# mattm458/tacotron2

Measured on AMD Instinct MI355X. Metric: mel-frames/sec (node), LJSpeech-shaped teacher-forced train step, b=32/GPU, fp32, higher is better.
Workload: dtype f32

## Files before the change

### include/tacotron2_amd.h

```cpp
#ifndef TACOTRON2_AMD_H
#define TACOTRON2_AMD_H
#include <stdint.h>
#ifdef __cplusplus
extern "C" {
#endif

#define T2_OK 0
#define T2_ERR_ARG 1
#define T2_ERR_LAUNCH 2
#define T2_ERR_RESIDENCY 3

const char* t2_last_error(void);
int t2_version(void);
int t2_sizeof(const char* struct_name);
int t2_debug_clock(int enable, uint64_t* out8);

typedef struct {
    const float* A; const float* B; float* C;
    int M, N, K;
    int64_t lda, ldb, ldc;
    int a_kmajor, b_kmajor;
    float alpha;
    const float* bias; const float* bias2;
    const float* mulmask; int64_t ldmask;
// ... 105 lines not shown
    const float* pre; const float* pmT; const float* memory; const int32_t* len;
    const float* att_drop;
    float* xdec; float* att_c; float* gates; float* align; float* cum; float* th;
    float* xproj_ctx; int64_t ld_xproj;
    float* e_part;
    int t_begin, t_end;
    float* xdec_t;
    uint64_t* clk;
} T2AttnSeq;
int t2_attn_seq_fwd(const T2AttnSeq* a, void* stream);

typedef struct {
    int B, L, T, A, Ad, Ef, Kl;
    const float* W_ih_ctx; int64_t ld_wih;
    const float* W_hh; const float* Wq; const float* U; const float* v;
    const float* wtp_ctx;
    const float* wtp_h;
    const float* wtp_q;
    const float* memory; const float* xdec; const float* att_c; const float* gates; const float* align;
    const float* cum; const float* th; const float* att_drop;
    const float* dh_ext; int64_t ld_dh;
    const float* dctx_ext1; int64_t ld_dc1;
    const float* dctx_ext2; int64_t ld_dc2;
    float* dgates; float* dctx_tot; float* dq; float* dpmT; float* dv_part; float* dU_part;
    float* dc; float* G; float* de; float* din_part;
    float* dh_rec;
    int t_hi, t_lo;
    float* dgates_t;
    uint64_t* clk;
    float* ws_bd;
    const float* dalign;
} T2AttnSeqBwd;
int t2_attn_seq_bwd(const T2AttnSeqBwd* a, void* stream);

int t2_embedding_fwd(const int64_t* idx, const float* table, float* out, int B, int L, int E, int pad, void* stream);
int t2_embedding_bwd(const int64_t* idx, const float* dout, float* dtable, int B, int L, int E, int Lp, int pad, void* stream);
int t2_pack_conv_weight(const float* w, float* wp, int Co, int Ci, int K, int flip, void* stream);
int t2_unpack_conv_wgrad(const float* gp, float* g, int Co, int Ci, int K, void* stream);

typedef struct {
    int B, L, C;
    const float* x; int Lp_x;
    const float* gamma; const float* beta;
    float* running_mean; float* running_var;
    int training; float momentum, eps;
    double* sums;
    float* mean; float* invstd;
    int act;
    const float* drop;
    const float* res; int Lp_res, pad_res;
    const int32_t* len; float fill;
    float* y; int Lp_y, pad_y;
    const float* dy; int Lp_dy, pad_dy;
    float* dx; int Lp_dx, pad_dx;
    float* dgamma; float* dbeta;
    int phase; const float* shift; float grad_share;
    int sums_prezeroed;
    const float* tile_stats; int tile_M;
} T2Bn;
int t2_bn_fwd(const T2Bn* s, void* stream);
int t2_bn_bwd(const T2Bn* s, void* stream);

int t2_colsum(const float* x, int64_t ld, int64_t R, int C, float* out, void* stream);
int t2_mel_to_tm(const float* mel, float* out, int B, int T, int M, void* stream);
int t2_swap01(const float* in, float* out, int D0, int D1, int C, int accumulate, void* stream);
int t2_finalize_fwd(const float* proj, int64_t ld_proj, const int32_t* len, float* mels, float* gates, float* post_in, int B,
// ... 65 lines not shown
```

### tacotron2_amd/csrc/t2_attention.hip

```cpp
#include "t2_common.hpp"
#include "t2_lstm_step.hpp"

int t2_lstm_step_fwd_launch(const T2LstmStep* steps, int n, hipStream_t st);
int t2_lstm_step_bwd_launch(const T2LstmBwdStep* steps, int n, hipStream_t st, unsigned long long* clk = nullptr);
void t2_lstm_fwd_advance(T2LstmStep& c, const T2LstmStride& inc);
void t2_lstm_bwd_advance(T2LstmBwdStep& c, const T2LstmBwdStride& inc);

namespace {

constexpr int KL = 31, KPAD = 15;

struct AttnK {
    int B, L, A, Ad, Ef;
    const float* att_h; long ldh;
    const float* Wq; const float* U; const float* v;
    const float* w_prev; long ldw; const float* cum_prev; long ldcum;
    const float* pmT; const float* memory; const int32_t* len;
    float* e_part; float* th_out;
    float* w_out; long ldwo; float* cum_out; long ldco;
    float* ctx_out; long ldctx; float* ctx_out2; long ldctx2;
    float* ctxt_out; int ctxt_col0; long ctxt_cs;
    unsigned long long* clk;
    int win_back, win_fwd; int32_t* win_peak;
};
// ... 618 lines not shown
        memset(&q, 0, sizeof(q));
        q.B = B; q.L = L; q.A = A; q.Ad = Ad; q.Ef = Ef; q.Kl = a->Kl;
        q.att_h = slot1; q.ldh = ldx; q.Wq = a->Wq; q.U = a->U; q.v = a->v;
        if (t > 0) { q.w_prev = a->align + (long)(t - 1) * L; q.ldw = (long)T * L; }
        q.cum_prev = a->cum + (long)t * B * L; q.ldcum = L;
        q.pmT = a->pmT; q.memory = a->memory; q.len = a->len; q.e_part = a->e_part;
        if (a->th) q.th_out = a->th + (long)t * B * Ad * ((L + 3) & ~3);
        q.w_out = a->align + (long)t * L; q.ldwo = (long)T * L;
        q.cum_out = a->cum + (long)(t + 1) * B * L; q.ldco = L;
        q.ctx_out = slot1 + A; q.ldctx = ldx;
        if (a->xproj_ctx) { q.ctx_out2 = a->xproj_ctx + (long)t * B * a->ld_xproj; q.ldctx2 = a->ld_xproj; }
        if (a->xdec_t) { q.ctxt_out = a->xdec_t + (long)(t + 1) * xts; q.ctxt_col0 = A; }
        q.clk = a->clk;
        if (t == tb) T2_TRY(check_attn(q));
        T2_TRY(launch_attn(q, st));
    }
    return T2_OK;
}

struct AttnBwdK {
    int B, L, Ad, Ef;
    const float* dctx; long lddctx;
    const float* ctx; long ldctx;
    const float* w; long ldw;
    const float* memory;
    const float* din_part; const float* G_in; float* G_out;
    const float* dalign;
    float* de;
    const float* th; const float* v; const float* U;
    const float* w_prev; long ldwp; const float* cum_prev; long ldcp;
    float* dpmT; float* dq; long lddq; float* dv_part; float* dU_part; float* din_part_out;
    unsigned long long* clk;
    const unsigned* bd;
};

namespace {

__global__ __launch_bounds__(256, 1) void attn_bwd_dw_kernel(AttnBwdK p) {
    T2_CHAIN_PRIO();
    extern __shared__ __attribute__((aligned(16))) float sm[];
    const int b = blockIdx.x, l0 = blockIdx.y * 32, tid = threadIdx.x;
    const int L = p.L, Ef = p.Ef, NA = p.Ad >> 4;
    constexpr int NEV = 20;
    const int DS = imax(Ef, 32 * NEV);
    float* dctx_s = sm;
    float* dwx_s = dctx_s + DS;
    float* red = dwx_s + ((L + 3) & ~3);
    [[maybe_unused]] const bool stamp = b == 0 && blockIdx.y == 0 && tid == 0;
    T2_STAMP(p, stamp, 16);
    T2_RING_BEGIN(p.clk, stamp, 3);
    const int l = l0 + (tid >> 3), sub = tid & 7;
    float dv0[4], cv0[4];
#pragma unroll
    for (int i = 0; i < 4; ++i) {
        const int e = imin(tid + 256 * i, Ef - 1);
        dv0[i] = p.dctx[(long)b * p.lddctx + e];
        cv0[i] = p.ctx[(long)b * p.ldctx + e];
    }
    const int lc0 = imin(tid, L - 1);
    float a0[8], a1[8];
#pragma unroll
    for (int jj = 0; jj < 8; ++jj) { a0[jj] = 0.f; a1[jj] = 0.f; }
    if (p.din_part) {
#pragma unroll
        for (int jj = 0; jj < 8; ++jj) {
            const long o = (((long)b * NA + imin(jj, NA - 1)) * 2) * L + lc0;
// ... 96 lines not shown
}

constexpr int DSH = 25;
constexpr int DS_ONE = 252;
constexpr int DS_TI = 216;
constexpr int DS_MARGIN = 16;

__global__ void attn_bwd_prep_kernel(const float* U, unsigned* bd, int Ad) {
    const int j = blockIdx.x, ks = blockIdx.y, lane = threadIdx.x, n = lane & 15, q = lane >> 4;
    const int blk = 4 * ks + q, al = blk / 5, rb = blk - 5 * al, c = n >> 3, sft = n & 7;
    float v[8];
#pragma unroll
    for (int jj = 0; jj < 8; ++jj) {
        const int k = 32 - (8 * rb + jj) + sft;
        v[jj] = (k >= 0 && k < KL) ? U[((long)(j * 16 + al) * 2 + c) * KL + k] : 0.f;
    }
    const Split8 sp = t2_split8(v);
    u32x4v* o = reinterpret_cast<u32x4v*>(bd) + ((long)(j * 20 + ks) * 3) * 64 + lane;
    o[0] = __builtin_bit_cast(u32x4v, sp.h); o[64] = __builtin_bit_cast(u32x4v, sp.m); o[128] = __builtin_bit_cast(u32x4v, sp.l);
}

struct DsDims { int NG, L4, M8, MT, KS, S16, LpI; };
__host__ __device__ inline DsDims ds_dims(int L) {
    DsDims d;
    d.NG = (L + 3) >> 2; d.L4 = 4 * d.NG; d.M8 = (L + 7) >> 3; d.MT = (d.M8 + 15) >> 4; d.KS = (L + 31) >> 5;
    int g = d.M8 + 5;
    if (4 * d.KS + 4 > g) g = 4 * d.KS + 4;
    if ((DSH + d.L4 + 7) / 8 + 1 > g) g = (DSH + d.L4 + 7) / 8 + 1;
    d.S16 = g | 1;
    d.LpI = 32 * d.KS + 96;
    return d;
}

template <bool TILED>
__device__ __forceinline__ void attn_bwd_ds_mfma_body(const AttnBwdK& p, float* sm) {
    const int b = blockIdx.x, j = blockIdx.y;
    const int tid = threadIdx.x, lane = tid & 63;
    [[maybe_unused]] const bool stamp = b == 0 && j == 0 && tid == 0;
    T2_STAMP(p, stamp, 24);
    T2_RING_BEGIN(p.clk, stamp, 4);
    const int w = __builtin_amdgcn_readfirstlane(tid >> 6);
    const int al = tid >> 5, sub = tid & 31, a = j * 16 + al;
    const int n = lane & 15, q = lane >> 4;
    const int Lg = p.L, Lg4 = (Lg + 3) & ~3;
    const DsDims dm = ds_dims(TILED ? imin(Lg, DS_TI + 2 * DS_MARGIN) : Lg);
    const int S16 = dm.S16, LpI = dm.LpI;
    u32x4v* DX = reinterpret_cast<u32x4v*>(sm);
    unsigned* PX = reinterpret_cast<unsigned*>(DX + 48 * S16);
    float* des = reinterpret_cast<float*>(PX + 6 * LpI);
    float* redC = des + dm.L4 + 8;
    float* dinacc = redC + 4 * 256;
    float* red = reinterpret_cast<float*>(DX);
    const long rowoff = ((long)b * p.Ad + a) * Lg;
    const float va = p.v[a];
    const float* th_base = p.th + ((long)b * p.Ad + a) * Lg4;
    const int c_nt = w & 3, c_c = c_nt >> 1, c_k = 16 * (c_nt & 1) + n;
    float sq = 0.f, sv = 0.f;
    f32x4 ch0 = {0.f, 0.f, 0.f, 0.f}, cl0 = ch0, cl1 = ch0, cl2 = ch0;
    u32x4v bdv[3][3];
    float dv_old = 0.f, dU_old[4] = {0.f, 0.f, 0.f, 0.f};
    const int ntile = TILED ? (Lg + DS_TI - 1) / DS_TI : 1;
    if (TILED) {
        for (int i = tid; i < 2 * Lg4; i += ENT) dinacc[i] = 0.f;
    }
    for (int tile = 0; tile < ntile; ++tile) {
        const int a0 = TILED ? tile * DS_TI : 0, b0 = TILED ? imin(a0 + DS_TI, Lg) : Lg;
        const int v0 = TILED ? imax(a0 - DS_MARGIN, 0) : 0, v1 = TILED ? imin(b0 + DS_MARGIN, Lg) : Lg;
        const int L = v1 - v0, ia = a0 - v0, ib = b0 - v0;
        const DsDims dd = TILED ? ds_dims(L) : dm;
        const int L4 = dd.L4, M8 = dd.M8, MT = dd.MT, KS = dd.KS;
        const int NGA = (L + 4) >> 2;
        float dev[TILED ? 1 : 2];
#pragma unroll
        for (int i = 0; i < (TILED ? 1 : 2); ++i) dev[i] = p.de[(long)b * Lg + v0 + imin(tid + ENT * i, L - 1)];
        float thv[EMAXI][4], dpv[EMAXI][4];
        const float* th_row = th_base + v0;
#pragma unroll
        for (int it = 0; it < EMAXI; ++it) {
            const int g = imin(sub + 32 * it, NGA - 1);
            const f32x4 t4 = *reinterpret_cast<const f32x4*>(th_row + imin(4 * g, L4 - 4));
            thv[it][0] = th_row[imax(4 * g - 1, 0)];
            thv[it][1] = t4[0]; thv[it][2] = t4[1]; thv[it][3] = t4[2];
        }
#pragma unroll
        for (int it = 0; it < EMAXI; ++it) {
            const int g = imin(sub + 32 * it, NGA - 1);
#pragma unroll
            for (int i = 0; i < 4; ++i) dpv[it][i] = p.dpmT[rowoff + v0 + imin(imax(4 * g - 1 + i, 0), L - 1)];
        }
        if (tile == 0) dv_old = p.dv_part[(long)b * p.Ad + a];
        StageRegs<ENT> sr;
        stage_issue<ENT, true, false>(sr, p.w_prev, p.ldwp, p.cum_prev, p.ldcp, p.U, p.dpmT, b, j, Lg, LpI, tid, 40, v0);
        if (tile == 0) {
            const u32x4v* bdp = reinterpret_cast<const u32x4v*>(p.bd) + (long)j * 20 * 3 * 64 + lane;
#pragma unroll
            for (int ki = 0; ki < 3; ++ki) {
                const int ks = imin(w + 8 * ki, 19);
#pragma unroll
                for (int pl = 0; pl < 3; ++pl) bdv[ki][pl] = bdp[(ks * 3 + pl) * 64];
            }
        }
        for (int i = tid; i < 48 * S16; i += ENT) DX[i] = (u32x4v){0u, 0u, 0u, 0u};
        stage_commit_split<ENT, false>(sr, PX, nullptr, p.w_prev, p.ldwp, p.cum_prev, p.ldcp, p.dpmT, b, Lg, LpI, tid, 40, v0);
#pragma unroll
        for (int i = 0; i < (TILED ? 1 : 2); ++i) {
            const int l = tid + ENT * i;
            if (l < dm.L4 + 7) des[l + 1] = (l >= ia && l < ib) ? dev[i] : 0.f;
        }
        if (tid == 0) des[0] = 0.f;
        __syncthreads();
        T2_STAMP(p, stamp, 25);

        {
            uint2* dx64 = reinterpret_cast<uint2*>(DX);
#pragma unroll
            for (int it = 0; it < EMAXI; ++it) {
                const int g = sub + 32 * it;
                if (g >= NGA) continue;
                f32x4 d4 = {0.f, 0.f, 0.f, 0.f};
                const f32x4 de4 = *reinterpret_cast<const f32x4*>(des + 4 * g);
#pragma unroll
                for (int i = 0; i < 4; ++i) {
                    const int l = 4 * g - 1 + i;
                    if (l >= ia && l < ib) {
                        const float th = thv[it][i];
                        d4[i] = de4[i] * va * (1.f - th * th);
                        sv += de4[i] * th;
                        p.dpmT[rowoff + v0 + l] = dpv[it][i] + d4[i];
                    }
                }
                sq += (d4[0] + d4[1]) + (d4[2] + d4[3]);
                const Split3 s3 = split3_attn(d4);
                const int o = al * S16 * 2 + 6 + g;
                dx64[o] = s3.h; dx64[16 * S16 * 2 + o] = s3.m; dx64[32 * S16 * 2 + o] = s3.l;
            }
        }
        if (!TILED) {
            sq = t2_half_sum_hi(sq); sv = t2_half_sum_hi(sv);
            if (sub == 31) {
                p.dq[(long)b * p.lddq + a] = sq;
                p.dv_part[(long)b * p.Ad + a] = dv_old + sv;
            }
        }
        __syncthreads();
        T2_STAMP(p, stamp, 26);
        if (tile == 0 && w < 4 && c_k < KL) {
#pragma unroll
            for (int r = 0; r < 4; ++r) dU_old[r] = p.dU_part[(((long)b * p.Ad + j * 16 + 4 * q + r) * 2 + c_c) * KL + c_k];
        }

        for (int ks = w >> 2; ks < KS + 1; ks += 2) {
            const int it = n * S16 + 4 * ks + q;
            Split8 fa, fb;
            fa.h = __builtin_bit_cast(bf16x8, DX[it]); fa.m = __builtin_bit_cast(bf16x8, DX[16 * S16 + it]); fa.l = __builtin_bit_cast(bf16x8, DX[32 * S16 + it]);
            const unsigned* bp = PX + c_c * LpI + 32 * ks + 8 * q + c_k;
            fb.h = __builtin_bit_cast(bf16x8, (u32x4v){bp[0], bp[2], bp[4], bp[6]});
            fb.m = __builtin_bit_cast(bf16x8, (u32x4v){bp[2 * LpI], bp[2 * LpI + 2], bp[2 * LpI + 4], bp[2 * LpI + 6]});
            fb.l = __builtin_bit_cast(bf16x8, (u32x4v){bp[4 * LpI], bp[4 * LpI + 2], bp[4 * LpI + 4], bp[4 * LpI + 6]});
            cl0 = __builtin_amdgcn_mfma_f32_16x16x32_bf16(fa.l, fb.h, cl0, 0, 0, 0);
            cl1 = __builtin_amdgcn_mfma_f32_16x16x32_bf16(fa.h, fb.l, cl1, 0, 0, 0);
            cl2 = __builtin_amdgcn_mfma_f32_16x16x32_bf16(fa.m, fb.m, cl2, 0, 0, 0);
            cl0 = __builtin_amdgcn_mfma_f32_16x16x32_bf16(fa.m, fb.h, cl0, 0, 0, 0);
            cl1 = __builtin_amdgcn_mfma_f32_16x16x32_bf16(fa.h, fb.m, cl1, 0, 0, 0);
            ch0 = __builtin_amdgcn_mfma_f32_16x16x32_bf16(fa.h, fb.h, ch0, 0, 0, 0);
        }
        if (!TILED && w >= 4) {
            const f32x4 cC1 = ch0 + ((cl0 + cl1) + cl2);
#pragma unroll
            for (int r = 0; r < 4; ++r) redC[c_nt * 256 + (4 * q + r) * 16 + n] = cC1[r];
        }
        T2_STAMP(p, stamp, 28);
        f32x4 cD[2];
#pragma unroll
        for (int mt = 0; mt < 2; ++mt) {
            f32x4 h0 = {0.f, 0.f, 0.f, 0.f}, l0 = h0, l1 = h0, l2 = h0;
            if (mt < MT) {
                const int m = imin(16 * mt + n, M8 - 1);
#pragma unroll
                for (int ki = 0; ki < 3; ++ki) {
                    const int ks = w + 8 * ki;
                    if (ks < 20) {
                        const int blk = 4 * ks + q, ad = blk / 5, rb = blk - 5 * ad;
                        const int it = ad * S16 + m + rb + 1;
                        Split8 fa, fb;
                        fa.h = __builtin_bit_cast(bf16x8, DX[it]); fa.m = __builtin_bit_cast(bf16x8, DX[16 * S16 + it]); fa.l = __builtin_bit_cast(bf16x8, DX[32 * S16 + it]);
                        fb.h = __builtin_bit_cast(bf16x8, bdv[ki][0]); fb.m = __builtin_bit_cast(bf16x8, bdv[ki][1]); fb.l = __builtin_bit_cast(bf16x8, bdv[ki][2]);
                        l0 = __builtin_amdgcn_mfma_f32_16x16x32_bf16(fa.l, fb.h, l0, 0, 0, 0);
                        l1 = __builtin_amdgcn_mfma_f32_16x16x32_bf16(fa.h, fb.l, l1, 0, 0, 0);
                        l2 = __builtin_amdgcn_mfma_f32_16x16x32_bf16(fa.m, fb.m, l2, 0, 0, 0);
                        l0 = __builtin_amdgcn_mfma_f32_16x16x32_bf16(fa.m, fb.h, l0, 0, 0, 0);
                        l1 = __builtin_amdgcn_mfma_f32_16x16x32_bf16(fa.h, fb.m, l1, 0, 0, 0);
                        h0 = __builtin_amdgcn_mfma_f32_16x16x32_bf16(fa.h, fb.h, h0, 0, 0, 0);
                    }
                }
            }
            cD[mt] = h0 + ((l0 + l1) + l2);
        }
        __syncthreads();
        T2_STAMP(p, stamp, 27);
#pragma unroll
        for (int mt = 0; mt < 2; ++mt) {
            if (mt < MT) {
#pragma unroll
                for (int r = 0; r < 4; ++r) red[((w * MT + mt) * 16 + 4 * q + r) * 16 + n] = cD[mt][r];
            }
        }
        if (!TILED && w < 4 && c_k < KL) {
            const f32x4 cC0 = ch0 + ((cl0 + cl1) + cl2);
#pragma unroll
            for (int r = 0; r < 4; ++r)
                p.dU_part[(((long)b * p.Ad + j * 16 + 4 * q + r) * 2 + c_c) * KL + c_k] = dU_old[r] + cC0[r] + redC[c_nt * 256 + (4 * q + r) * 16 + n];
        }
        __syncthreads();
        T2_STAMP(p, stamp, 29);
        for (int o = tid; o < MT * 256; o += ENT) {
            const int mt = o >> 8, ml = (o >> 4) & 15, nn = o & 15;
            float s2 = 0.f;
#pragma unroll
            for (int ww = 0; ww < 8; ++ww) s2 += red[((ww * MT + mt) * 16 + ml) * 16 + nn];
            const int m = 16 * mt + ml, l = 8 * m + (nn & 7);
            if (m < M8 && l < L) {
                if (TILED) dinacc[(nn >> 3) * Lg4 + v0 + l] += s2;
                else p.din_part_out[(((long)b * (p.Ad >> 4) + j) * 2 + (nn >> 3)) * Lg + l] = s2;
            }
        }
        if (TILED) __syncthreads();
    }
    if (TILED) {
        sq = t2_half_sum_hi(sq); sv = t2_half_sum_hi(sv);
        if (sub == 31) {
            p.dq[(long)b * p.lddq + a] = sq;
            p.dv_part[(long)b * p.Ad + a] = dv_old + sv;
        }
    }
    if (TILED) {
        const f32x4 cC = ch0 + ((cl0 + cl1) + cl2);
        if (w >= 4) {
#pragma unroll
            for (int r = 0; r < 4; ++r) redC[c_nt * 256 + (4 * q + r) * 16 + n] = cC[r];
        }
        __syncthreads();
        if (w < 4 && c_k < KL) {
#pragma unroll
            for (int r = 0; r < 4; ++r)
                p.dU_part[(((long)b * p.Ad + j * 16 + 4 * q + r) * 2 + c_c) * KL + c_k] = dU_old[r] + cC[r] + redC[c_nt * 256 + (4 * q + r) * 16 + n];
        }
    }
    if (TILED) {
        for (int i = tid; i < 2 * Lg; i += ENT) {
            const int c = i >= Lg ? 1 : 0, l = i - c * Lg;
            p.din_part_out[(((long)b * (p.Ad >> 4) + j) * 2 + c) * Lg + l] = dinacc[c * Lg4 + l];
        }
    }
    T2_STAMP(p, stamp, 30);
    T2_RING_END();
}

__global__ __launch_bounds__(ENT, 4) void attn_bwd_ds_mfma_kernel(AttnBwdK p) {
    T2_CHAIN_PRIO();
    extern __shared__ __attribute__((aligned(16))) float sm[];
    attn_bwd_ds_mfma_body<false>(p, sm);
}
__global__ __launch_bounds__(ENT, 2) void attn_bwd_ds_tiled_kernel(AttnBwdK p) {
    T2_CHAIN_PRIO();
    extern __shared__ __attribute__((aligned(16))) float sm[];
    attn_bwd_ds_mfma_body<true>(p, sm);
}

size_t ds_mfma_lds(int L) {
    const bool tiled = L > DS_ONE;
    const DsDims dd = ds_dims(tiled ? (L < DS_TI + 2 * DS_MARGIN ? L : DS_TI + 2 * DS_MARGIN) : L);
    size_t f = (size_t)48 * dd.S16 * 4 + 6 * dd.LpI + dd.L4 + 8 + 4 * 256;
    if (tiled) f += (size_t)2 * ((L + 3) & ~3);
    return f * sizeof(float);
}

}

extern "C" int t2_attn_seq_bwd(const T2AttnSeqBwd* a, void* stream) {
    (void)hipGetLastError();
    T2_REQUIRE(a != nullptr, "t2_attn_seq_bwd: null");
    T2_REQUIRE(a->Kl == KL && a->Ad % 16 == 0 && a->Ef % 32 == 0, "t2_attn_seq_bwd: unsupported dims");
    T2_REQUIRE(a->L >= 1, "t2_attn_seq_bwd: need L >= 1");
    T2_REQUIRE(a->ws_bd && a->th, "t2_attn_seq_bwd: the filter workspace ws_bd and the forward's tanh stash th are required");
    hipStream_t st = (hipStream_t)stream;
    const int B = a->B, L = a->L, T = a->T, A = a->A, Ef = a->Ef, Ad = a->Ad, NA = Ad / 16;
    const long ldx = A + Ef;
    const size_t sm_dw = (size_t)((Ef > 640 ? Ef : 640) + ((L + 3) & ~3) + 8) * sizeof(float);
    const bool tiled = L > DS_ONE;
    const size_t sm_dsm = ds_mfma_lds(L);
    T2_REQUIRE(t2_allow_lds(attn_bwd_dw_kernel, sm_dw) && (tiled ? t2_allow_lds(attn_bwd_ds_tiled_kernel, sm_dsm) : t2_allow_lds(attn_bwd_ds_mfma_kernel, sm_dsm)),
               "t2_attn_seq_bwd: the text is too long for the LDS images of the attention backward kernels");
    hipLaunchKernelGGL(attn_bwd_prep_kernel, dim3(NA, 20), dim3(64), 0, st, a->U, reinterpret_cast<unsigned*>(a->ws_bd), Ad);
    T2_REQUIRE(a->wtp_ctx && a->wtp_h, "t2_attn_seq_bwd: packed weight streams (t2_lstm_pack_bwd) are required");
    const long ldz = 4 * A + Ad;
    float* Z = a->dgates;
    T2_REQUIRE(a->wtp_q && a->dh_rec, "t2_attn_seq_bwd: wtp_q / dh_rec required");
    T2_REQUIRE(!a->dgates_t || A % 16 == 0, "t2_attn_seq_bwd: dgates_t needs A % 16 == 0");
    const int thi = (a->t_hi == 0 && a->t_lo == 0) ? T : a->t_hi, tlo = (a->t_hi == 0 && a->t_lo == 0) ? 0 : a->t_lo;
    T2_REQUIRE(tlo >= 0 && thi <= T && tlo <= thi, "t2_attn_seq_bwd: bad frame range");
    T2LstmBwdStep s2[2];
    for (int t = thi - 1; t >= tlo; --t) {
        const bool last = (t == T - 1);
        const float* zrow = Z + (long)(t + 1) * B * ldz;
        memset(s2, 0, sizeof(s2));
        T2LstmBwdStep& s = s2[0];
        s.B = B; s.H = A; s.N4 = 4 * A; s.dg_next = zrow; s.lddg = ldz; s.W = a->W_ih_ctx; s.ldw = a->ld_wih;
        s.ncols = Ef; s.epi = 0; s.wtpacked = a->wtp_ctx;
        s.ext1 = a->dctx_ext1 + (long)t * B * a->ld_dc1; s.ldx1 = a->ld_dc1;
        s.ext2 = a->dctx_ext2 + (long)t * B * a->ld_dc2; s.ldx2 = a->ld_dc2;
        s.dx_out = a->dctx_tot + (long)t * B * Ef; s.lddx = Ef;
        const long zts = (long)(4 * A / 16) * ((B + 15) / 16 * 16) * 16;
        if (a->dgates_t) s.dgt_next = a->dgates_t + (long)(t + 1) * zts;
        T2LstmBwdStep& r = s2[1];
        r.B = B; r.H = A; r.N4 = 4 * A; r.dg_next = zrow; r.lddg = ldz; r.W = a->W_hh; r.ldw = A;
        r.ncols = A; r.epi = 0; r.wtpacked = a->wtp_h;
        r.ext1 = a->dh_ext + (long)t * B * a->ld_dh; r.ldx1 = a->ld_dh;
        r.dx_out = a->dh_rec; r.lddx = A;
        if (a->dgates_t) r.dgt_next = a->dgates_t + (long)(t + 1) * zts;
        T2_TRY(t2_lstm_step_bwd_launch(s2, 2, st, (unsigned long long*)a->clk));
        AttnBwdK k;
        memset(&k, 0, sizeof(k));
        k.B = B; k.L = L; k.Ad = Ad; k.Ef = Ef;
        k.dctx = a->dctx_tot + (long)t * B * Ef; k.lddctx = Ef;
        k.ctx = a->xdec + (long)(t + 1) * B * ldx + A; k.ldctx = ldx;
        k.w = a->align + (long)t * L; k.ldw = (long)T * L;
        k.memory = a->memory;
        k.din_part = last ? nullptr : a->din_part;
        k.G_in = last ? nullptr : a->G + (long)((t + 1) & 1) * B * L;
        k.G_out = a->G + (long)(t & 1) * B * L;
        k.dalign = a->dalign ? a->dalign + (long)t * L : nullptr;
        k.de = a->de;
        k.th = a->th + (long)t * B * Ad * ((L + 3) & ~3); k.v = a->v; k.U = a->U;
        if (t > 0) { k.w_prev = a->align + (long)(t - 1) * L; k.ldwp = (long)T * L; }
        k.cum_prev = a->cum + (long)t * B * L; k.ldcp = L;
        k.dpmT = a->dpmT; k.dq = Z + (long)(t + 1) * B * ldz + 4 * A; k.lddq = ldz;
        k.dv_part = a->dv_part; k.dU_part = a->dU_part; k.din_part_out = a->din_part;
        k.clk = (unsigned long long*)a->clk;
        hipLaunchKernelGGL(attn_bwd_dw_kernel, dim3(B, t2_cdiv(L, 32)), dim3(256), sm_dw, st, k);
        k.bd = reinterpret_cast<const unsigned*>(a->ws_bd);
        if (tiled) hipLaunchKernelGGL(attn_bwd_ds_tiled_kernel, dim3(B, NA), dim3(ENT), sm_dsm, st, k);
        else hipLaunchKernelGGL(attn_bwd_ds_mfma_kernel, dim3(B, NA), dim3(ENT), sm_dsm, st, k);
        T2LstmBwdStep c;
        memset(&c, 0, sizeof(c));
        c.B = B; c.H = A; c.N4 = Ad; c.dg_next = Z + (long)(t + 1) * B * ldz + 4 * A; c.lddg = ldz; c.W = a->Wq; c.ldw = A;
        c.ncols = A; c.epi = 1; c.wtpacked = a->wtp_q;
        c.ext1 = a->dh_rec; c.ldx1 = A;
        if (a->att_drop) { c.drop = a->att_drop + (long)t * B * A; c.lddrop = A; }
        c.gates = a->gates + (long)t * B * 4 * A; c.ldgs = 4 * A;
        c.c_prev = a->att_c + (long)t * B * A; c.ldcp = A;
        c.c_cur = a->att_c + (long)(t + 1) * B * A; c.ldcc = A;
        c.dc = a->dc; c.lddc = A;
        c.dg_out = Z + (long)t * B * ldz; c.ldgo = ldz;
        if (a->dgates_t) c.dgt_out = a->dgates_t + (long)t * zts;
        T2_TRY(t2_lstm_step_bwd_launch(&c, 1, st, (unsigned long long*)a->clk));
    }
    T2_CHECK_LAUNCH();
    return T2_OK;
}
```

### tacotron2_amd/engine.py

```python
from __future__ import annotations

import contextlib
import numbers
import threading as _threading
from typing import Dict, Optional

import torch

from . import _lib
from . import guard as _guard
from ._lib import call, make
from .params import ParamStore

KL, KPAD = 31, 15


def _stream():
    return torch.cuda.current_stream().cuda_stream


_TLS = _threading.local()


@contextlib.contextmanager
# ... 845 lines not shown
        def proj_wgrads():
            self._wgrad(dproj, M + 1, _ptr(xproj, B * ldp), ldp, ps.cat_view("decoder.mel_out.weight", M + 1, ldp, grad=True),
                        ldp, M + 1, ldp, R)
            call("t2_colsum", dproj, M + 1, R, M + 1, ps.cat_view("decoder.mel_out.bias", M + 1, 0, grad=True), _stream())
            if ctl is not None:
                C = ctl.shape[1]
                s_proj = self.buf("ctl.dproj_sum", B, M + 1, zero=True)
                call("t2_colsum", dproj, B * (M + 1), T, B * (M + 1), s_proj, _stream())
                self._wgrad(s_proj, M + 1, ctl, C, G["decoder.mel_out.weight#controls"], C, M, C, B)
        post_wgrads.append(proj_wgrads)

        dgd = self.buf("dgd", T + 1, B, 4 * D)
        zero_later(dgd[T])
        Bp = (B + 15) // 16 * 16
        dgd_t = self.buf("dgd_t", T + 1, 4 * D // 16, Bp, 16)
        zero_later(dgd_t[T])
        Zt = self.buf("Zatt_t", T + 1, 4 * A // 16, Bp, 16)
        zero_later(Zt[T])
        dc_dec = self.buf("dc_dec", B, D, zero=True)
        dd = masks.get("dec_drop")
        wtp_dec = self.pack_bwd("dec.t", P["decoder.lstm.weight_hh"], D, 4 * D, D)
        dxdec = self.buf("dxdec", T, B, ldx)
        ldz = 4 * A + Ad
        Z = self.buf("Zatt", T + 1, B, ldz)
        zero_later(Z[T, :, :4 * A])
        dga = Z
        dctx_tot = self.buf("dctx_tot", T, B, Ef)
        dpmT = self.buf("dpmT", B, Ad, L, zero=True)
        dv_part = self.buf("dv_part", B, Ad, zero=True)
        dU_part = self.buf("dU_part", B, Ad * 2 * KL, zero=True)
        dc_att = self.buf("dc_att", B, A, zero=True)
        Gc = self.buf("Gcum", 2, B, L)
        de = self.buf("de", B, L)
        din_part = self.buf("din_part", B, Ad // 16, 2, L)
        wtp_ctx = self.pack_bwd("att.ctx.t", _ptr(P["decoder.att_rnn.weight_ih"], Pd), Pd + Ef, 4 * A, Ef)
        wtp_h = self.pack_bwd("att.h.t", P["decoder.att_rnn.weight_hh"], A, 4 * A, A)
        wtp_q = self.pack_bwd("att.q.t", P["decoder.attention.query_layer.weight"], A, Ad, A)
        dh_rec = self.buf("dh_rec", B, A)
        sb = make("T2AttnSeqBwd", B=B, L=L, T=T, A=A, Ad=Ad, Ef=Ef, Kl=KL, wtp_ctx=wtp_ctx, wtp_h=wtp_h, wtp_q=wtp_q,
                  dh_rec=dh_rec,
                  W_ih_ctx=_ptr(P["decoder.att_rnn.weight_ih"], Pd), ld_wih=Pd + Ef, W_hh=P["decoder.att_rnn.weight_hh"],
                  Wq=P["decoder.attention.query_layer.weight"], U=ctx["U"], v=P["decoder.attention.v.weight"],
                  memory=ctx["memory"], xdec=xdec, att_c=ctx["att_c"], gates=ctx["gates_att"], align=ctx["align"],
                  cum=ctx["cum"], th=ctx["th"], att_drop=masks.get("att_drop"),
                  dh_ext=dxdec, ld_dh=ldx, dctx_ext1=_ptr(dxdec, A), ld_dc1=ldx, dctx_ext2=_ptr(dxproj, D), ld_dc2=ldp,
                  dgates=Z, dctx_tot=dctx_tot, dq=None, dpmT=dpmT, dv_part=dv_part, dU_part=dU_part,
                  dc=dc_att, G=Gc, de=de, din_part=din_part, dgates_t=Zt, clk=getattr(self, "clk_bwd", None), dalign=d_align,
                  ws_bd=self.buf("attn.ws_bd", Ad // 16 * 16896))
        self.mark("bwd.dec.proj")
        main, side = torch.cuda.current_stream(), self.side_stream()
        self._wait(side, main)
        CH = self.chunk_bwd

        def dec_bwd_chunk(hi, lo):
            s = make("T2LstmBwdStep", B=B, H=D, N4=4 * D, dg_next=_ptr(dgd, hi * B * 4 * D), lddg=4 * D,
                     W=P["decoder.lstm.weight_hh"], ldw=D, wtpacked=wtp_dec, ncols=D, epi=1,
                     ext1=_ptr(dxproj, (hi - 1) * B * ldp), ldx1=ldp,
                     drop=_ptr(dd, (hi - 1) * B * D) if dd is not None else None, lddrop=D,
                     gates=_ptr(ctx["gates_dec"], (hi - 1) * B * 4 * D), ldgs=4 * D,
                     c_prev=_ptr(ctx["dec_c"], (hi - 1) * B * D), ldcp=D, c_cur=_ptr(ctx["dec_c"], hi * B * D), ldcc=D,
                     dc=dc_dec, lddc=D, dg_out=_ptr(dgd, (hi - 1) * B * 4 * D), ldgo=4 * D,
                     dgt_next=_ptr(dgd_t, hi * Bp * 4 * D), dgt_out=_ptr(dgd_t, (hi - 1) * Bp * 4 * D),
                     off_chain=1 if self.bptt_off_chain else 0)
            inc = make("T2LstmBwdStride", dg=-B * 4 * D, ext1=-B * ldp, drop=-B * D, gates=-B * 4 * D, c_prev=-B * D,
                       c_cur=-B * D, dt=0, dgt=-Bp * 4 * D)
            return s, inc

        def dec_wgrads_chunk(hi, lo):
            n = (hi - lo) * B
            g0 = _ptr(dgd, lo * B * 4 * D)
            self._wgrad(g0, 4 * D, _ptr(xdec, (lo + 1) * B * ldx), ldx, G["decoder.lstm.weight_ih"], ldx, 4 * D, ldx, n)
            self._wgrad(g0, 4 * D, _ptr(xproj, lo * B * ldp), ldp, G["decoder.lstm.weight_hh"], D, 4 * D, D, n)

        chunks, hi = [], T
        for n in reversed(_chunk_sizes(T, CH, ramp_at_end=self.ramp_chunks)):
            chunks.append((hi, hi - n)); hi -= n
        gWih = G["decoder.att_rnn.weight_ih"]

        def att_wgrads(hi, lo):
            n = (hi - lo) * B
            z0 = _ptr(Z, lo * B * ldz)
            self._wgrad(z0, ldz, _ptr(ctx["p2"], lo * B * Pd), Pd, gWih, Pd + Ef, 4 * A, Pd, n)
            self._wgrad(z0, ldz, _ptr(xdec, lo * B * ldx + A), ldx, _ptr(gWih, Pd), Pd + Ef, 4 * A, Ef, n)
            self._wgrad(z0, ldz, _ptr(xdec, lo * B * ldx), ldx, G["decoder.att_rnn.weight_hh"], A, 4 * A, A, n)
            self._wgrad(_ptr(Z, (lo + 1) * B * ldz + 4 * A), ldz, _ptr(xdec, (lo + 1) * B * ldx), ldx,
                        G["decoder.attention.query_layer.weight"], A, Ad, A, n)
        WG = max(1, int(self.wgrad_group))
        dec_grp, att_done, att_grp = None, [], None
        for ci_, (hi, lo) in enumerate(chunks):
            with torch.cuda.stream(side), share_cu(self.share_cu):
                s, inc = dec_bwd_chunk(hi, lo)
                call("t2_lstm_seq_bwd", s, inc, 1, hi - lo, side.cuda_stream)
                gemm(_ptr(dgd, lo * B * 4 * D), P["decoder.lstm.weight_ih"], _ptr(dxdec, lo * B * ldx), (hi - lo) * B, ldx, 4 * D,
                     4 * D, ldx, ldx, a_k=1, b_k=0)
                ev = self._record(side)
                dec_grp = [hi, lo, 1] if dec_grp is None else [dec_grp[0], lo, dec_grp[2] + 1]
                if dec_grp[2] >= WG:
                    dec_wgrads_chunk(dec_grp[0], dec_grp[1]); dec_grp = None
                if post_wgrads and ci_ >= 4:
                    post_wgrads.pop(0)()
                if len(att_done) >= 2:
                    h2, l2, e2 = att_done.pop(0)
                    att_grp = [h2, l2, 1, e2] if att_grp is None else [att_grp[0], l2, att_grp[2] + 1, e2]
                    if att_grp[2] >= WG:
                        self._wait(side, att_grp[3])
                        att_wgrads(att_grp[0], att_grp[1]); att_grp = None
            self._wait(main, ev)
            sb.t_hi, sb.t_lo = hi, lo
            call("t2_attn_seq_bwd", sb, st)
            att_done.append((hi, lo, self._record(main)))
        with torch.cuda.stream(side):
            while post_wgrads:
                post_wgrads.pop(0)()
            with share_cu(self.share_cu):
                if dec_grp is not None:
                    dec_wgrads_chunk(dec_grp[0], dec_grp[1])
                for h2, l2, e2 in att_done:
                    att_grp = [h2, l2, 1, e2] if att_grp is None else [att_grp[0], l2, att_grp[2] + 1, e2]
                if att_grp is not None:
                    self._wait(side, att_grp[3])
                    att_wgrads(att_grp[0], att_grp[1])
            db = self.buf("db_dec", 4 * D, zero=True)
            call("t2_colsum", dgd, 4 * D, R, 4 * D, db, side.cuda_stream)
            for nm in ("decoder.lstm.bias_ih", "decoder.lstm.bias_hh"):
                call("t2_colsum", db, 4 * D, 1, 4 * D, G[nm], side.cuda_stream)
            if ctl is not None:
                s_dgd = self.buf("ctl.dgd_sum", B, 4 * D, zero=True)
                call("t2_colsum", dgd, B * 4 * D, T, B * 4 * D, s_dgd, side.cuda_stream)
                self._wgrad(s_dgd, 4 * D, ctl, ctl.shape[1], G["decoder.lstm.weight_ih#controls"], ctl.shape[1], 4 * D,
                            ctl.shape[1], B)
        self.mark("bwd.dec.chains")

        dmem = self.buf("dmem", B, L, Ef)
        gemm(ctx["align"], dctx_tot, dmem, L, Ef, T, L, B * Ef, Ef, a_k=0, b_k=0, batch=B, sA=T * L, sB=Ef, sC=L * Ef)
        Watt = P["att_encoder.weight"]
        gemm(dpmT, Watt, dmem, L, Ef, Ad, L, Ef, Ef, a_k=0, b_k=0, accumulate=1, batch=B, sA=Ad * L, sB=0, sC=L * Ef)

        self._wait(side, main)
        with torch.cuda.stream(side):
            sst = side.cuda_stream
            db = self.buf("db_att", 4 * A, zero=True)
            call("t2_colsum", dga, ldz, R, 4 * A, db, sst)
            for nm in ("decoder.att_rnn.bias_ih", "decoder.att_rnn.bias_hh"):
                call("t2_colsum", db, 4 * A, 1, 4 * A, G[nm], sst)
            call("t2_colsum", dv_part, Ad, B, Ad, G["decoder.attention.v.weight"], sst)
            dU = self.buf("dU", Ad, 2 * KL, zero=True)
            call("t2_colsum", dU_part, Ad * 2 * KL, B, Ad * 2 * KL, dU, sst)
            Wd, Wc = P["decoder.attention.location_dense.weight"], P["decoder.attention.location_conv.weight"]
            gemm(dU, Wc, G["decoder.attention.location_dense.weight"], Ad, F, 2 * KL, 2 * KL, 2 * KL, F, accumulate=1)
            gemm(Wd, dU, G["decoder.attention.location_conv.weight"], F, 2 * KL, Ad, F, 2 * KL, 2 * KL, a_k=0, b_k=0,
                 accumulate=1)
            gemm(dpmT, ctx["memory"], G["att_encoder.weight"], Ad, Ef, L, L, Ef, Ef, a_k=1, b_k=0, accumulate=2, batch=B,
                 sA=Ad * L, sB=L * Ef, sC=0)
            dp2 = self.buf("dp2", T + 1, B, Pd)
            zero_later(dp2[T])
            gemm(dga, P["decoder.att_rnn.weight_ih"], dp2, R, Pd, 4 * A, ldz, Pd + Ef, Pd, a_k=1, b_k=0)
            pd = ctx["pd"]
            g2 = self.buf("g2", T + 1, B, Pd)
            call("t2_relu_mask_bwd", dp2, ctx["p2"], pd[1] if pd else None, g2, R1 * Pd, sst)
            self._wgrad(g2, Pd, ctx["p1"], Pd, G["prenet.3.weight"], Pd, Pd, Pd, R1)
            dp1 = self.buf("dp1", T + 1, B, Pd)
            gemm(g2, P["prenet.3.weight"], dp1, R1, Pd, Pd, Pd, Pd, Pd, a_k=1, b_k=0)
            g1 = self.buf("g1", T + 1, B, Pd)
            call("t2_relu_mask_bwd", dp1, ctx["p1"], pd[0] if pd else None, g1, R1 * Pd, sst)
            self._wgrad(g1, Pd, ctx["mel_tm"], M, G["prenet.0.weight"], M, Pd, M, R1)
            if self.grad_tail_hook is not None:
                self.grad_tail_hook()
        self.mark("bwd.dec.attn_gemms")
# ... 250 lines not shown
```

Measured before the change: 291,900.

## Split attention backward into chain-critical part and deferred side-stream accumulation

The per-frame attention backward kernel on the serial chain is split. A lighter chain variant computes only the recurrence-critical outputs (dq and the location-gradient path) and stashes the per-frame energy gradients. The non-critical accumulations (dpmT, dv, dU) are done later by a new kernel that walks frame ranges on the side stream, overlapping the decoder chain. This shortens the serial critical path and uses less LDS per chain block, at the cost of a T×B×L stash buffer, extra memory traffic, and extra cross-stream waits.

After: 296,100 (median of 6 runs). 1.01x the previous value.

```diff
diff --git a/include/tacotron2_amd.h b/include/tacotron2_amd.h
--- a/include/tacotron2_amd.h
+++ b/include/tacotron2_amd.h
@@ -161,6 +161,9 @@
     const float* dalign;
 } T2AttnSeqBwd;
 int t2_attn_seq_bwd(const T2AttnSeqBwd* a, void* stream);
+
+int t2_attn_seq_bwd_stash(const T2AttnSeqBwd* a, float* de_stash, int64_t ld_stash, void* stream);
+int t2_attn_acc_bwd(const T2AttnSeqBwd* a, const float* de_stash, int64_t ld_stash, int t_begin, int t_end, void* stream);
 
 int t2_embedding_fwd(const int64_t* idx, const float* table, float* out, int B, int L, int E, int pad, void* stream);
 int t2_embedding_bwd(const int64_t* idx, const float* dout, float* dtable, int B, int L, int E, int Lp, int pad, void* stream);
diff --git a/tacotron2_amd/csrc/t2_attention.hip b/tacotron2_amd/csrc/t2_attention.hip
--- a/tacotron2_amd/csrc/t2_attention.hip
+++ b/tacotron2_amd/csrc/t2_attention.hip
@@ -674,6 +674,7 @@
     float* dpmT; float* dq; long lddq; float* dv_part; float* dU_part; float* din_part_out;
     unsigned long long* clk;
     const unsigned* bd;
+    int t_begin, t_end; long de_fs, th_fs, cum_fs, w_fs;
 };
 
 namespace {
@@ -836,11 +837,15 @@
     return d;
 }
 
-template <bool TILED>
+enum { DS_FULL = 0, DS_CHAIN = 1, DS_ACC = 2 };
+
+template <bool TILED, int MODE>
 __device__ __forceinline__ void attn_bwd_ds_mfma_body(const AttnBwdK& p, float* sm) {
+    constexpr bool ACC = MODE != DS_CHAIN, CHN = MODE != DS_ACC, WALK = MODE == DS_ACC;
+    static_assert(!TILED || MODE == DS_FULL, "position tiles accumulate in the chain");
     const int b = blockIdx.x, j = blockIdx.y;
     const int tid = threadIdx.x, lane = tid & 63;
-    [[maybe_unused]] const bool stamp = b == 0 && j == 0 && tid == 0;
+    [[maybe_unused]] const bool stamp = !WALK && b == 0 && j == 0 && tid == 0;
     T2_STAMP(p, stamp, 24);
     T2_RING_BEGIN(p.clk, stamp, 4);
     const int w = __builtin_amdgcn_readfirstlane(tid >> 6);
@@ -851,13 +856,14 @@
     const int S16 = dm.S16, LpI = dm.LpI;
     u32x4v* DX = reinterpret_cast<u32x4v*>(sm);
     unsigned* PX = reinterpret_cast<unsigned*>(DX + 48 * S16);
-    float* des = reinterpret_cast<float*>(PX + 6 * LpI);
+    float* des = reinterpret_cast<float*>(PX + (ACC ? 6 * LpI : 0));
     float* redC = des + dm.L4 + 8;
     float* dinacc = redC + 4 * 256;
     float* red = reinterpret_cast<float*>(DX);
     const long rowoff = ((long)b * p.Ad + a) * Lg;
     const float va = p.v[a];
     const float* th_base = p.th + ((long)b * p.Ad + a) * Lg4;
+    float dpv[EMAXI][4];
     const int c_nt = w & 3, c_c = c_nt >> 1, c_k = 16 * (c_nt & 1) + n;
     float sq = 0.f, sv = 0.f;
     f32x4 ch0 = {0.f, 0.f, 0.f, 0.f}, cl0 = ch0, cl1 = ch0, cl2 = ch0;
@@ -867,18 +873,40 @@
     if (TILED) {
         for (int i = tid; i < 2 * Lg4; i += ENT) dinacc[i] = 0.f;
     }
-    for (int tile = 0; tile < ntile; ++tile) {
+    if (WALK) {
+#pragma unroll
+        for (int it = 0; it < EMAXI; ++it)
+#pragma unroll
+            for (int i = 0; i < 4; ++i) dpv[it][i] = 0.f;
+        for (int i = tid; i < 48 * S16; i += ENT) DX[i] = (u32x4v){0u, 0u, 0u, 0u};
+    }
+    const int nwalk = WALK ? p.t_end - p.t_begin : ntile;
+    for (int tile = 0; tile < nwalk; ++tile) {
+        const int fr = WALK ? p.t_end - 1 - tile : 0;
+        const float* de_fr = WALK ? p.de + fr * p.de_fs : p.de;
+        const float* w_prev = WALK ? (fr > 0 ? p.w + (fr - 1) * p.w_fs : nullptr) : p.w_prev;
+        const float* cum_prev = WALK ? p.cum_prev + fr * p.cum_fs : p.cum_prev;
         const int a0 = TILED ? tile * DS_TI : 0, b0 = TILED ? imin(a0 + DS_TI, Lg) : Lg;
         const int v0 = TILED ? imax(a0 - DS_MARGIN, 0) : 0, v1 = TILED ? imin(b0 + DS_MARGIN, Lg) : Lg;
         const int L = v1 - v0, ia = a0 - v0, ib = b0 - v0;
         const DsDims dd = TILED ? ds_dims(L) : dm;
         const int L4 = dd.L4, M8 = dd.M8, MT = dd.MT, KS = dd.KS;
         const int NGA = (L + 4) >> 2;
-        float dev[TILED ? 1 : 2];
-#pragma unroll
-        for (int i = 0; i < (TILED ? 1 : 2); ++i) dev[i] = p.de[(long)b * Lg + v0 + imin(tid + ENT * i, L - 1)];
-        float thv[EMAXI][4], dpv[EMAXI][4];
-        const float* th_row = th_base + v0;
+        float dev[TILED ? 1 : 2], dew[EMAXI][4];
+        if (!WALK) {
+#pragma unroll
+            for (int i = 0; i < (TILED ? 1 : 2); ++i) dev[i] = de_fr[(long)b * Lg + v0 + imin(tid + ENT * i, L - 1)];
+        }
+        float thv[EMAXI][4];
+        const float* th_row = th_base + (WALK ? fr * p.th_fs : 0) + v0;
+        if (WALK) {
+#pragma unroll
+            for (int it = 0; it < EMAXI; ++it) {
+                const int g = imin(sub + 32 * it, NGA - 1);
+#pragma unroll
+                for (int i = 0; i < 4; ++i) dew[it][i] = de_fr[(long)b * Lg + imin(imax(4 * g - 1 + i, 0), L - 1)];
+            }
+        }
 #pragma unroll
         for (int it = 0; it < EMAXI; ++it) {
             const int g = imin(sub + 32 * it, NGA - 1);
@@ -886,16 +914,18 @@
             thv[it][0] = th_row[imax(4 * g - 1, 0)];
             thv[it][1] = t4[0]; thv[it][2] = t4[1]; thv[it][3] = t4[2];
         }
-#pragma unroll
-        for (int it = 0; it < EMAXI; ++it) {
-            const int g = imin(sub + 32 * it, NGA - 1);
-#pragma unroll
-            for (int i = 0; i < 4; ++i) dpv[it][i] = p.dpmT[rowoff + v0 + imin(imax(4 * g - 1 + i, 0), L - 1)];
-        }
-        if (tile == 0) dv_old = p.dv_part[(long)b * p.Ad + a];
+        if (MODE == DS_FULL) {
+#pragma unroll
+            for (int it = 0; it < EMAXI; ++it) {
+                const int g = imin(sub + 32 * it, NGA - 1);
+#pragma unroll
+                for (int i = 0; i < 4; ++i) dpv[it][i] = p.dpmT[rowoff + v0 + imin(imax(4 * g - 1 + i, 0), L - 1)];
+            }
+            if (tile == 0) dv_old = p.dv_part[(long)b * p.Ad + a];
+        }
         StageRegs<ENT> sr;
-        stage_issue<ENT, true, false>(sr, p.w_prev, p.ldwp, p.cum_prev, p.ldcp, p.U, p.dpmT, b, j, Lg, LpI, tid, 40, v0);
-        if (tile == 0) {
+        if (ACC) stage_issue<ENT, true, false>(sr, w_prev, p.ldwp, cum_prev, p.ldcp, p.U, p.dpmT, b, j, Lg, LpI, tid, 40, v0);
+        if (CHN && tile == 0) {
             const u32x4v* bdp = reinterpret_cast<const u32x4v*>(p.bd) + (long)j * 20 * 3 * 64 + lane;
 #pragma unroll
             for (int ki = 0; ki < 3; ++ki) {
@@ -904,15 +934,21 @@
                 for (int pl = 0; pl < 3; ++pl) bdv[ki][pl] = bdp[(ks * 3 + pl) * 64];
             }
         }
-        for (int i = tid; i < 48 * S16; i += ENT) DX[i] = (u32x4v){0u, 0u, 0u, 0u};
-        stage_commit_split<ENT, false>(sr, PX, nullptr, p.w_prev, p.ldwp, p.cum_prev, p.ldcp, p.dpmT, b, Lg, LpI, tid, 40, v0);
-#pragma unroll
-        for (int i = 0; i < (TILED ? 1 : 2); ++i) {
-            const int l = tid + ENT * i;
-            if (l < dm.L4 + 7) des[l + 1] = (l >= ia && l < ib) ? dev[i] : 0.f;
-        }
-        if (tid == 0) des[0] = 0.f;
-        __syncthreads();
+        if (WALK) {
+            __syncthreads();
+        } else {
+            for (int i = tid; i < 48 * S16; i += ENT) DX[i] = (u32x4v){0u, 0u, 0u, 0u};
+        }
+        if (ACC) stage_commit_split<ENT, false>(sr, PX, nullptr, w_prev, p.ldwp, cum_prev, p.ldcp, p.dpmT, b, Lg, LpI, tid, 40, v0);
+        if (!WALK) {
+#pragma unroll
+            for (int i = 0; i < (TILED ? 1 : 2); ++i) {
+                const int l = tid + ENT * i;
+                if (l < dm.L4 + 7) des[l + 1] = (l >= ia && l < ib) ? dev[i] : 0.f;
+            }
+            if (tid == 0) des[0] = 0.f;
+            __syncthreads();
+        }
         T2_STAMP(p, stamp, 25);
 
         {
@@ -922,38 +958,42 @@
                 const int g = sub + 32 * it;
                 if (g >= NGA) continue;
                 f32x4 d4 = {0.f, 0.f, 0.f, 0.f};
-                const f32x4 de4 = *reinterpret_cast<const f32x4*>(des + 4 * g);
+                f32x4 de4;
+                if (WALK) de4 = (f32x4){dew[it][0], dew[it][1], dew[it][2], dew[it][3]};
+                else de4 = *reinterpret_cast<const f32x4*>(des + 4 * g);
 #pragma unroll
                 for (int i = 0; i < 4; ++i) {
                     const int l = 4 * g - 1 + i;
                     if (l >= ia && l < ib) {
                         const float th = thv[it][i];
                         d4[i] = de4[i] * va * (1.f - th * th);
-                        sv += de4[i] * th;
-                        p.dpmT[rowoff + v0 + l] = dpv[it][i] + d4[i];
+                        if (ACC) sv += de4[i] * th;
+                        if (MODE == DS_FULL) p.dpmT[rowoff + v0 + l] = dpv[it][i] + d4[i];
+                        if (WALK) dpv[it][i] += d4[i];
                     }
                 }
-                sq += (d4[0] + d4[1]) + (d4[2] + d4[3]);
+                if (CHN) sq += (d4[0] + d4[1]) + (d4[2] + d4[3]);
                 const Split3 s3 = split3_attn(d4);
                 const int o = al * S16 * 2 + 6 + g;
                 dx64[o] = s3.h; dx64[16 * S16 * 2 + o] = s3.m; dx64[32 * S16 * 2 + o] = s3.l;
             }
         }
-        if (!TILED) {
-            sq = t2_half_sum_hi(sq); sv = t2_half_sum_hi(sv);
+        if (!TILED && CHN) {
+            sq = t2_half_sum_hi(sq);
+            if (MODE == DS_FULL) sv = t2_half_sum_hi(sv);
             if (sub == 31) {
                 p.dq[(long)b * p.lddq + a] = sq;
-                p.dv_part[(long)b * p.Ad + a] = dv_old + sv;
+                if (MODE == DS_FULL) p.dv_part[(long)b * p.Ad + a] = dv_old + sv;
             }
         }
         __syncthreads();
         T2_STAMP(p, stamp, 26);
-        if (tile == 0 && w < 4 && c_k < KL) {
+        if (MODE == DS_FULL && tile == 0 && w < 4 && c_k < KL) {
 #pragma unroll
             for (int r = 0; r < 4; ++r) dU_old[r] = p.dU_part[(((long)b * p.Ad + j * 16 + 4 * q + r) * 2 + c_c) * KL + c_k];
         }
 
-        for (int ks = w >> 2; ks < KS + 1; ks += 2) {
+        for (int ks = w >> 2; ACC && ks < KS + 1; ks += 2) {
             const int it = n * S16 + 4 * ks + q;
             Split8 fa, fb;
             fa.h = __builtin_bit_cast(bf16x8, DX[it]); fa.m = __builtin_bit_cast(bf16x8, DX[16 * S16 + it]); fa.l = __builtin_bit_cast(bf16x8, DX[32 * S16 + it]);
@@ -968,12 +1008,13 @@
             cl1 = __builtin_amdgcn_mfma_f32_16x16x32_bf16(fa.h, fb.m, cl1, 0, 0, 0);
             ch0 = __builtin_amdgcn_mfma_f32_16x16x32_bf16(fa.h, fb.h, ch0, 0, 0, 0);
         }
-        if (!TILED && w >= 4) {
+        if (MODE == DS_FULL && !TILED && w >= 4) {
             const f32x4 cC1 = ch0 + ((cl0 + cl1) + cl2);
 #pragma unroll
             for (int r = 0; r < 4; ++r) redC[c_nt * 256 + (4 * q + r) * 16 + n] = cC1[r];
         }
         T2_STAMP(p, stamp, 28);
+        if (WALK) continue;
         f32x4 cD[2];
 #pragma unroll
         for (int mt = 0; mt < 2; ++mt) {
@@ -1009,7 +1050,7 @@
                 for (int r = 0; r < 4; ++r) red[((w * MT + mt) * 16 + 4 * q + r) * 16 + n] = cD[mt][r];
             }
         }
-        if (!TILED && w < 4 && c_k < KL) {
+        if (MODE == DS_FULL && !TILED && w < 4 && c_k < KL) {
             const f32x4 cC0 = ch0 + ((cl0 + cl1) + cl2);
 #pragma unroll
             for (int r = 0; r < 4; ++r)
@@ -1037,7 +1078,26 @@
             p.dv_part[(long)b * p.Ad + a] = dv_old + sv;
         }
     }
-    if (TILED) {
+    if (WALK) {
+        sv = t2_half_sum_hi(sv);
+        if (sub == 31) p.dv_part[(long)b * p.Ad + a] += sv;
+        const int NGA = (Lg + 4) >> 2;
+#pragma unroll
+        for (int it = 0; it < EMAXI; ++it) {
+            const int g = sub + 32 * it;
+            if (g >= NGA) continue;
+#pragma unroll
+            for (int i = 0; i < 4; ++i) {
+                const int l = 4 * g - 1 + i;
+                if (l >= 0 && l < Lg) p.dpmT[rowoff + l] += dpv[it][i];
+            }
+        }
+        if (w < 4 && c_k < KL) {
+#pragma unroll
+            for (int r = 0; r < 4; ++r) dU_old[r] = p.dU_part[(((long)b * p.Ad + j * 16 + 4 * q + r) * 2 + c_c) * KL + c_k];
+        }
+    }
+    if (TILED || WALK) {
         const f32x4 cC = ch0 + ((cl0 + cl1) + cl2);
         if (w >= 4) {
 #pragma unroll
@@ -1063,25 +1123,36 @@
 __global__ __launch_bounds__(ENT, 4) void attn_bwd_ds_mfma_kernel(AttnBwdK p) {
     T2_CHAIN_PRIO();
     extern __shared__ __attribute__((aligned(16))) float sm[];
-    attn_bwd_ds_mfma_body<false>(p, sm);
+    attn_bwd_ds_mfma_body<false, DS_FULL>(p, sm);
+}
+__global__ __launch_bounds__(ENT, 4) void attn_bwd_ds_chain_kernel(AttnBwdK p) {
+    T2_CHAIN_PRIO();
+    extern __shared__ __attribute__((aligned(16))) float sm[];
+    attn_bwd_ds_mfma_body<false, DS_CHAIN>(p, sm);
+}
+__global__ __launch_bounds__(ENT, 4) void attn_bwd_acc_kernel(AttnBwdK p) {
+    extern __shared__ __attribute__((aligned(16))) float sm[];
+    attn_bwd_ds_mfma_body<false, DS_ACC>(p, sm);
 }
 __global__ __launch_bounds__(ENT, 2) void attn_bwd_ds_tiled_kernel(AttnBwdK p) {
     T2_CHAIN_PRIO();
     extern __shared__ __attribute__((aligned(16))) float sm[];
-    attn_bwd_ds_mfma_body<true>(p, sm);
-}
-
-size_t ds_mfma_lds(int L) {
+    attn_bwd_ds_mfma_body<true, DS_FULL>(p, sm);
+}
+
+size_t ds_mfma_lds(int L, int mode = DS_FULL) {
     const bool tiled = L > DS_ONE;
     const DsDims dd = ds_dims(tiled ? (L < DS_TI + 2 * DS_MARGIN ? L : DS_TI + 2 * DS_MARGIN) : L);
-    size_t f = (size_t)48 * dd.S16 * 4 + 6 * dd.LpI + dd.L4 + 8 + 4 * 256;
+    size_t f = (size_t)48 * dd.S16 * 4 + dd.L4 + 8;
+    if (mode != DS_CHAIN) f += 6 * dd.LpI + 4 * 256;
+    if (f < (size_t)8 * dd.MT * 256) f = (size_t)8 * dd.MT * 256;
     if (tiled) f += (size_t)2 * ((L + 3) & ~3);
     return f * sizeof(float);
 }
 
 }
 
-extern "C" int t2_attn_seq_bwd(const T2AttnSeqBwd* a, void* stream) {
+static int attn_seq_bwd(const T2AttnSeqBwd* a, float* de_stash, long ld_stash, void* stream) {
     (void)hipGetLastError();
     T2_REQUIRE(a != nullptr, "t2_attn_seq_bwd: null");
     T2_REQUIRE(a->Kl == KL && a->Ad % 16 == 0 && a->Ef % 32 == 0, "t2_attn_seq_bwd: unsupported dims");
@@ -1092,8 +1163,10 @@
     const long ldx = A + Ef;
     const size_t sm_dw = (size_t)((Ef > 640 ? Ef : 640) + ((L + 3) & ~3) + 8) * sizeof(float);
     const bool tiled = L > DS_ONE;
-    const size_t sm_dsm = ds_mfma_lds(L);
-    T2_REQUIRE(t2_allow_lds(attn_bwd_dw_kernel, sm_dw) && (tiled ? t2_allow_lds(attn_bwd_ds_tiled_kernel, sm_dsm) : t2_allow_lds(attn_bwd_ds_mfma_kernel, sm_dsm)),
+    if (tiled) de_stash = nullptr;
+    T2_REQUIRE(!de_stash || ld_stash >= (long)B * L, "t2_attn_seq_bwd_stash: ld_stash < B * L");
+    const size_t sm_dsm = ds_mfma_lds(L, de_stash ? DS_CHAIN : DS_FULL);
+    T2_REQUIRE(t2_allow_lds(attn_bwd_dw_kernel, sm_dw) && (tiled ? t2_allow_lds(attn_bwd_ds_tiled_kernel, sm_dsm) : de_stash ? t2_allow_lds(attn_bwd_ds_chain_kernel, sm_dsm) : t2_allow_lds(attn_bwd_ds_mfma_kernel, sm_dsm)),
                "t2_attn_seq_bwd: the text is too long for the LDS images of the attention backward kernels");
     hipLaunchKernelGGL(attn_bwd_prep_kernel, dim3(NA, 20), dim3(64), 0, st, a->U, reinterpret_cast<unsigned*>(a->ws_bd), Ad);
     T2_REQUIRE(a->wtp_ctx && a->wtp_h, "t2_attn_seq_bwd: packed weight streams (t2_lstm_pack_bwd) are required");
@@ -1134,7 +1207,7 @@
         k.G_in = last ? nullptr : a->G + (long)((t + 1) & 1) * B * L;
         k.G_out = a->G + (long)(t & 1) * B * L;
         k.dalign = a->dalign ? a->dalign + (long)t * L : nullptr;
-        k.de = a->de;
+        k.de = de_stash ? de_stash + (long)t * ld_stash : a->de;
         k.th = a->th + (long)t * B * Ad * ((L + 3) & ~3); k.v = a->v; k.U = a->U;
         if (t > 0) { k.w_prev = a->align + (long)(t - 1) * L; k.ldwp = (long)T * L; }
         k.cum_prev = a->cum + (long)t * B * L; k.ldcp = L;
@@ -1144,6 +1217,7 @@
         hipLaunchKernelGGL(attn_bwd_dw_kernel, dim3(B, t2_cdiv(L, 32)), dim3(256), sm_dw, st, k);
         k.bd = reinterpret_cast<const unsigned*>(a->ws_bd);
         if (tiled) hipLaunchKernelGGL(attn_bwd_ds_tiled_kernel, dim3(B, NA), dim3(ENT), sm_dsm, st, k);
+        else if (de_stash) hipLaunchKernelGGL(attn_bwd_ds_chain_kernel, dim3(B, NA), dim3(ENT), sm_dsm, st, k);
         else hipLaunchKernelGGL(attn_bwd_ds_mfma_kernel, dim3(B, NA), dim3(ENT), sm_dsm, st, k);
         T2LstmBwdStep c;
         memset(&c, 0, sizeof(c));
@@ -1162,3 +1236,35 @@
     T2_CHECK_LAUNCH();
     return T2_OK;
 }
+
+extern "C" int t2_attn_seq_bwd(const T2AttnSeqBwd* a, void* stream) { return attn_seq_bwd(a, nullptr, 0, stream); }
+
+extern "C" int t2_attn_seq_bwd_stash(const T2AttnSeqBwd* a, float* de_stash, int64_t ld_stash, void* stream) {
+    return attn_seq_bwd(a, de_stash, (long)ld_stash, stream);
+}
+
+extern "C" int t2_attn_acc_bwd(const T2AttnSeqBwd* a, const float* de_stash, int64_t ld_stash, int t_begin, int t_end, void* stream) {
+    (void)hipGetLastError();
+    T2_REQUIRE(a != nullptr && de_stash != nullptr, "t2_attn_acc_bwd: null");
+    T2_REQUIRE(a->Kl == KL && a->Ad % 16 == 0 && a->L >= 1, "t2_attn_acc_bwd: unsupported dims");
+    T2_REQUIRE(a->th && a->align && a->cum && a->v && a->dpmT && a->dv_part && a->dU_part, "t2_attn_acc_bwd: null operand");
+    T2_REQUIRE(t_begin >= 0 && t_end <= a->T && t_begin <= t_end, "t2_attn_acc_bwd: bad frame range");
+    const int B = a->B, L = a->L, Ad = a->Ad;
+    T2_REQUIRE(ld_stash >= (long)B * L, "t2_attn_acc_bwd: ld_stash < B * L");
+    if (L > DS_ONE || t_begin == t_end) return T2_OK;
+    const size_t smem = ds_mfma_lds(L, DS_ACC);
+    T2_REQUIRE(t2_allow_lds(attn_bwd_acc_kernel, smem), "t2_attn_acc_bwd: LDS");
+    AttnBwdK k;
+    memset(&k, 0, sizeof(k));
+    k.B = B; k.L = L; k.Ad = Ad; k.Ef = a->Ef;
+    k.t_begin = t_begin; k.t_end = t_end;
+    k.de = const_cast<float*>(de_stash); k.de_fs = (long)ld_stash;
+    k.th = a->th; k.th_fs = (long)B * Ad * ((L + 3) & ~3);
+    k.v = a->v; k.U = a->U;
+    k.w = a->align; k.w_fs = L; k.ldwp = (long)a->T * L;
+    k.cum_prev = a->cum; k.cum_fs = (long)B * L; k.ldcp = L;
+    k.dpmT = a->dpmT; k.dv_part = a->dv_part; k.dU_part = a->dU_part;
+    hipLaunchKernelGGL(attn_bwd_acc_kernel, dim3(B, Ad / 16), dim3(ENT), smem, (hipStream_t)stream, k);
+    T2_CHECK_LAUNCH();
+    return T2_OK;
+}
diff --git a/tacotron2_amd/engine.py b/tacotron2_amd/engine.py
--- a/tacotron2_amd/engine.py
+++ b/tacotron2_amd/engine.py
@@ -901,6 +901,7 @@
         dc_att = self.buf("dc_att", B, A, zero=True)
         Gc = self.buf("Gcum", 2, B, L)
         de = self.buf("de", B, L)
+        de_stash = self.buf("de_stash", T, B, L) if L <= 252 else None
         din_part = self.buf("din_part", B, Ad // 16, 2, L)
         wtp_ctx = self.pack_bwd("att.ctx.t", _ptr(P["decoder.att_rnn.weight_ih"], Pd), Pd + Ef, 4 * A, Ef)
         wtp_h = self.pack_bwd("att.h.t", P["decoder.att_rnn.weight_hh"], A, 4 * A, A)
@@ -956,6 +957,12 @@
                         G["decoder.attention.query_layer.weight"], A, Ad, A, n)
         WG = max(1, int(self.wgrad_group))
         dec_grp, att_done, att_grp = None, [], None
+
+        def att_acc(hi, lo, ev):
+            if de_stash is None:
+                return
+            self._wait(side, ev)
+            call("t2_attn_acc_bwd", sb, de_stash, B * L, lo, hi, side.cuda_stream)
         for ci_, (hi, lo) in enumerate(chunks):
             with torch.cuda.stream(side), share_cu(self.share_cu):
                 s, inc = dec_bwd_chunk(hi, lo)
@@ -970,20 +977,25 @@
                     post_wgrads.pop(0)()
                 if len(att_done) >= 2:
                     h2, l2, e2 = att_done.pop(0)
+                    att_acc(h2, l2, e2)
                     att_grp = [h2, l2, 1, e2] if att_grp is None else [att_grp[0], l2, att_grp[2] + 1, e2]
                     if att_grp[2] >= WG:
                         self._wait(side, att_grp[3])
                         att_wgrads(att_grp[0], att_grp[1]); att_grp = None
             self._wait(main, ev)
             sb.t_hi, sb.t_lo = hi, lo
-            call("t2_attn_seq_bwd", sb, st)
+            call("t2_attn_seq_bwd_stash", sb, de_stash, B * L, st)
             att_done.append((hi, lo, self._record(main)))
         with torch.cuda.stream(side):
+            for h2, l2, e2 in att_done[:-1]:
+                att_acc(h2, l2, e2)
             while post_wgrads:
                 post_wgrads.pop(0)()
             with share_cu(self.share_cu):
                 if dec_grp is not None:
                     dec_wgrads_chunk(dec_grp[0], dec_grp[1])
+                att_acc(*att_done[-1])
+                acc_done = self._record(side)
                 for h2, l2, e2 in att_done:
                     att_grp = [h2, l2, 1, e2] if att_grp is None else [att_grp[0], l2, att_grp[2] + 1, e2]
                 if att_grp is not None:
@@ -1003,6 +1015,7 @@
         dmem = self.buf("dmem", B, L, Ef)
         gemm(ctx["align"], dctx_tot, dmem, L, Ef, T, L, B * Ef, Ef, a_k=0, b_k=0, batch=B, sA=T * L, sB=Ef, sC=L * Ef)
         Watt = P["att_encoder.weight"]
+        self._wait(main, acc_done)
         gemm(dpmT, Watt, dmem, L, Ef, Ad, L, Ef, Ef, a_k=0, b_k=0, accumulate=1, batch=B, sA=Ad * L, sB=0, sC=L * Ef)
 
         self._wait(side, main)
```
